# Tai-Wang/Depth-from-Motion

Hardware: AMD Instinct MI355X
Metric: cost-volumes/sec (higher is better)
Workload: dtype bf16; 1 GPU; nstar: plane-sweep cost-volume build B=8/GPU x (2C=512, D=112, 94x311), feats 256x94x311 bf16, fsf=4 csf=1; global_batch=8, parallelism=dp1, kernel=sweep_tile_kernel<LDS>, launch=lanes256_ppl8_planes2_chunk1_pipelined_cut64, autotuned=True, volume_layout=(B,2C,D,H,W) contiguous (the reference layout)

## Files before the change

### depth-from-motion_amd/_capi.py

```python
import ctypes
import os

_HERE = os.path.dirname(os.path.abspath(__file__))
LIB_PATH = os.environ.get('DFM_HIP_LIB', os.path.join(_HERE, 'lib', 'libdfm_hip.so'))

DFM_F32, DFM_BF16 = 0, 1


class SweepDesc(ctypes.Structure):
    _fields_ = [
        ('batch', ctypes.c_int32),
        ('channels', ctypes.c_int32),
        ('h_in', ctypes.c_int32),
        ('w_in', ctypes.c_int32),
        ('num_depths', ctypes.c_int32),
        ('h_out', ctypes.c_int32),
        ('w_out', ctypes.c_int32),
        ('feat_sample_factor', ctypes.c_float),
        ('cost_sample_factor', ctypes.c_float),
        ('img_scale_factor', ctypes.c_float),
        ('crop_x', ctypes.c_float),
        ('crop_y', ctypes.c_float),
        ('org_w', ctypes.c_float),
        ('flip', ctypes.c_int32),
        ('dtype', ctypes.c_int32),
    ]


class SweepOpts(ctypes.Structure):
    _fields_ = [(n, ctypes.c_int32) for n in (
        'kernel', 'lanes_per_workgroup', 'lds_kib', 'blocks_per_group', 'planes_per_workgroup',
        'bands_per_chunk', 'points_per_lane', 'pipeline', 'store_align_points', 'pair_stores',
        'unpack')] + [('reserved', ctypes.c_int32 * 1)]

    def as_dict(self):
        return {n: getattr(self, n) for n, _ in self._fields_ if n != 'reserved'}


class MvDesc(ctypes.Structure):
    _fields_ = [
        ('num_views', ctypes.c_int32),
        ('num_frames', ctypes.c_int32),
        ('channels', ctypes.c_int32),
        ('feat_h', ctypes.c_int32),
        ('feat_w', ctypes.c_int32),
        ('nx', ctypes.c_int32),
        ('ny', ctypes.c_int32),
        ('nz', ctypes.c_int32),
        ('num_points', ctypes.c_int64),
        ('scale_x', ctypes.c_float),
        ('scale_y', ctypes.c_float),
        ('crop_x', ctypes.c_float),
        ('crop_y', ctypes.c_float),
        ('flip', ctypes.c_int32),
        ('pad_h', ctypes.c_float),
        ('pad_w', ctypes.c_float),
        ('mode', ctypes.c_int32),
        ('aggregate', ctypes.c_int32),
        ('valid_sample', ctypes.c_int32),
        ('dtype', ctypes.c_int32),
        ('out_channels_last', ctypes.c_int32),
        ('feats_channels_last', ctypes.c_int32),
    ]


class F2vDesc(ctypes.Structure):
    _fields_ = [(n, ctypes.c_int32) for n in (
        'batch', 'channels', 'd', 'h', 'w', 'ds', 'hs', 'ws', 'sem_channels', 'hsem', 'wsem', 'nz',
        'ny', 'nx')] + [(n, ctypes.c_float) for n in ('pad_h', 'pad_w', 'depth_min', 'depth_span')
# ... 208 lines not shown
    ci, i32, i64, sz, f32, f64 = (ctypes.c_int, ctypes.c_int32, ctypes.c_int64, ctypes.c_size_t, ctypes.c_float,
                                  ctypes.c_double)
    dp, op, mp, f2p, spp, pp = P(SweepDesc), P(SweepOpts), P(MvDesc), P(F2vDesc), P(SppDesc), P(vp)
    vsp, vmp, cp, wp, lp = P(VsDesc), P(VsMvDesc), P(Conv3dDesc), P(Conv3dWgradDesc), P(DepthLossDesc)
    ip, atp, ahp, adp, ddp = P(ImitationDesc), P(AnchorTargetDesc), P(AnchorHeadDesc), P(AtssTargetDesc), P(DeformDesc)
    vdp, sdp, plp, i32p, i64p = P(VoxelDesc), P(SparseConvDesc), P(SparseConvPlan), P(i32), P(i64)
    dtp, alp, slp = P(DepthTargetsDesc), P(AnchorLossDesc), P(AtssLossDesc)
    return {
        'dfm_hip.h': _table(
            ('dfm_version', ci, []),
            ('dfm_last_error', ctypes.c_char_p, []),
            ('dfm_profile_begin', ci, [ci]),
            ('dfm_profile_end', ci, [P(f64), P(ci)]),
            ('dfm_camera_prepare', ci, [fp, i32, i32, i32, fp, fp, vp]),
            ('dfm_plane_sweep_workspace_bytes', sz, [dp]),
            ('dfm_plane_sweep_fwd', ci, [dp, vp, vp, fp, fp, fp, fp, vp, vp, sz, vp]),
            ('dfm_plane_sweep_cl_workspace_bytes', sz, [dp]),
            ('dfm_plane_sweep_fwd_channels_last', ci, [dp, vp, vp, fp, fp, fp, fp, vp, vp, sz, vp]),
            ('dfm_plane_sweep_fwd_nhwc', ci, [dp, vp, vp, fp, fp, fp, fp, vp, vp, sz, vp]),
            ('dfm_plane_sweep_fwd_from_nhwc', ci, [dp, vp, vp, fp, fp, fp, fp, vp, vp, sz, vp]),
            ('dfm_plane_sweep_bwd', ci, [dp, vp, fp, fp, fp, fp, fp, fp, vp]),
            ('dfm_plane_sweep_grid', ci, [dp, i32, fp, fp, fp, fp, fp, fp, vp]),
            ('dfm_plane_sweep_last_kernel', ci, []),
            ('dfm_plane_sweep_bwd_last_kernel', ci, []),
            ('dfm_plane_sweep_fwd_opts', ci, [dp, vp, vp, fp, fp, fp, fp, vp, vp, sz, vp, op]),
            ('dfm_plane_sweep_bwd_opts', ci, [dp, vp, fp, fp, fp, fp, fp, fp, vp, op]),
            ('dfm_plane_sweep_bwd_channels_last', ci, [dp, vp, fp, fp, fp, fp, fp, fp, vp, sz, vp]),
            ('dfm_plane_sweep_bwd_cur_nhwc', ci, [dp, vp, fp, fp, fp, fp, fp, vp]),
            ('dfm_plane_sweep_bwd_prev_gather_workspace_bytes', sz, [dp]),
            ('dfm_plane_sweep_bwd_prev_gather', ci, [dp, vp, fp, fp, fp, fp, fp, vp, sz, vp]),
            ('dfm_plane_sweep_bwd_gather', ci, [dp, i32, vp, i32, fp, fp, fp, fp, fp, i32, vp, sz, vp]),
            ('dfm_plane_sweep_autotune', ci, [dp, vp, vp, fp, fp, fp, fp, vp, vp, sz, vp, op]),
            ('dfm_plane_sweep_tuning', ci, [dp, op]),
            ('dfm_plane_sweep_reset_tuning', None, []),
            ('dfm_store_probe', ci, [vp, i32, i32, i64, i32, i32, vp]),
            ('dfm_clock_probe', ci, [vp, i32, vp]),
            ('dfm_point_sample_mv_workspace_bytes', sz, [mp]),
            ('dfm_point_sample_mv_fwd', ci, [mp, vp, fp, fp, fp, vp, vp, vp, sz, vp]),
            ('dfm_frustum_to_voxel_workspace_bytes', sz, [f2p]),
            ('dfm_frustum_to_voxel_fwd', ci, [f2p, vp, vp, vp, fp, fp, vp, vp, sz, vp]),
            ('dfm_depth_head_fwd', ci, [i32, i32, i32, i32, i32, i32, vp, fp, vp, vp, vp, vp]),
            ('dfm_depth_head_stats_fwd', ci, [i32, i32, i32, i32, i32, i32, vp, fp, fp, fp, vp, vp]),
            ('dfm_frustum_to_voxel_fused_fwd', ci, [f2p, vp, vp, fp, fp, i32, vp, fp, fp, vp, vp, sz, vp]),
            ('dfm_frustum_to_voxel_bwd_workspace_bytes', sz, [f2p]),
            ('dfm_frustum_to_voxel_bwd', ci, [f2p, vp, vp, fp, fp, fp, fp, vp, sz, vp]),
            ('dfm_frustum_to_voxel_fused_bwd', ci, [f2p, vp, vp, fp, fp, i32, fp, fp, fp, fp, vp, sz, vp]),
            ('dfm_frustum_to_voxel_bwd_gather_workspace_bytes', sz, [f2p]),
            ('dfm_frustum_to_voxel_bwd_gather', ci, [f2p, vp, vp, vp, fp, fp, i32, fp, P(f32), fp, fp, fp, vp, sz,
                                                     vp]),
            ('dfm_frustum_to_voxel_bwd_gather_cl', ci, [f2p, vp, vp, vp, fp, fp, i32, fp, P(f32), fp, vp, fp, vp, sz,
                                                        vp]),
            ('dfm_point_sample_mv_fwd_batched', ci, [vp, i32, vp, fp, i32, fp, fp, vp, vp, vp]),
            ('dfm_point_sample_mv_bwd_workspace_bytes', sz, [mp]),
            ('dfm_point_sample_mv_bwd', ci, [mp, vp, fp, fp, fp, fp, vp, sz, vp]),
            ('dfm_depth_head_bwd', ci, [i32, i32, i32, i32, i32, i32, vp, fp, vp, vp, vp, fp, vp]),
            ('dfm_sweep_conv_weight_bytes', sz, []),
            ('dfm_sweep_conv_pack_weights', ci, [vp, vp, i32, vp, vp]),
            ('dfm_sweep_conv_stats_splits', ci, [dp, i32]),
            ('dfm_sweep_conv_fwd', ci, [dp, vp, vp, fp, fp, fp, fp, vp, vp, vp, fp, fp, i32, vp]),
            ('dfm_cost_gate_weight_bytes', sz, [i32]),
            ('dfm_cost_gate_pack_weights', ci, [vp, i32, i32, vp, vp]),
            ('dfm_cost_gate_fwd', ci, [i32, i32, i64, i32, vp, vp, vp, vp, vp]),
            ('dfm_conv3d_k3_c32_weight_bytes', sz, []),
            ('dfm_conv3d_k3_c32_pack_weights', ci, [vp, i32, i32, i32, i32, vp, vp]),
            ('dfm_conv3d_k3_c32_stats_splits', ci, [i32, i32, i32, i32, i32]),
            ('dfm_conv3d_k3_c32_fwd', ci, [i32, i32, i32, i32, vp, vp, fp, vp, i32, i32, i32, fp, vp]),
# ... 179 lines not shown
```

### depth-from-motion_amd/csrc/plane_sweep.hip

```cpp
#include "plane_sweep_common.h"

#include <stdlib.h>
#include <string.h>

#include <algorithm>
#include <map>
#include <mutex>
#include <vector>

using namespace dfm;

namespace {

thread_local int g_last_kernel = 0;
#ifdef DFM_DEBUG_HOOKS
unsigned long long *g_trace = nullptr;
#endif

struct Launch {
    int kernel;
    int lanes;
    int lds_kib;
    int bpg;
    int planes;
    int band_chunk;
    int ppl;
    int align;
    int pair;
    int unpack;
    int pipe;
};

struct TuneKey {
    int v[9];
    bool operator<(const TuneKey &o) const { return memcmp(v, o.v, sizeof(v)) < 0; }
};
std::mutex g_tune_mu;
std::map<TuneKey, dfm_sweep_opts> g_tuned;

constexpr int PACK_PPL = 1;
__global__ void sweep_reset_kernel(int *flags, int n_flags, int *b, int *c)
{
    for (int i = threadIdx.x; i < n_flags; i += blockDim.x) flags[i] = 0;
    if (threadIdx.x == 0) { *b = 0; *c = 0; }
}

template <typename T>
__global__ __launch_bounds__(256) void pack_blocked_kernel(const T *__restrict__ src0,
                                                           const T *__restrict__ src1,
                                                           uint4 *__restrict__ dst0,
                                                           uint4 *__restrict__ dst1, int batch,
                                                           int C, int HW, int nblk, int *__restrict__ flags,
                                                           int W)
{
    constexpr int CB = elem<T>::CB;
    const int pix0 = blockIdx.x * (256 * PACK_PPL) + threadIdx.x;
    const int blk = blockIdx.y;
    const bool second = (int)blockIdx.z >= batch;
// ... 171 lines not shown
        dc += HW;
        dp += HW;
    }
}

typedef uint32_t u32x4_t __attribute__((ext_vector_type(4)));

__device__ __forceinline__ void vol_store16(const u32x4_t &v, void *p)
{
    __builtin_nontemporal_store(v, (u32x4_t *)p);
}

__device__ __forceinline__ constexpr int waitcnt_vm(int n)
{
    return (n & 15) | (7 << 4) | (15 << 8) | ((n >> 4) << 14);
}

__device__ __forceinline__ int swz(int q) { return q ^ ((q >> 4) & 7); }

__device__ __forceinline__ uint32_t footprint(float x, float y, int H, int W, int &rN, int &rS,
                                              int &ix, float &fw, float &fn)
{
    const Tap t = make_tap(x, y, H, W);
    ix = (t.ok & 5u) ? t.ix : t.ix - ((t.ok & 10u) ? 1 : 0);
    rN = t.iy;
    rS = t.iy + t.dy;
    const bool fin = (fabsf(x) <= 3.0e38f) && (fabsf(y) <= 3.0e38f);
    fw = fin ? x - floorf(x) : 0.0f;
    fn = fin ? y - floorf(y) : 0.0f;
    return t.ok;
}

struct TileGrid {
    int batch;
    int bands;
    int band_pts;
    int planes;
    int dgroups;
    int blocks_per_group;
    int band_chunk;
    const int *flags;
    int mfma_unpack;
    int pair_stores;
    int align;
    unsigned long long *trace;
    int ablate;
};

constexpr int PIPE_BUF_SLOTS = 2504;
constexpr int PIPE_LDS_BYTES = (8 + 2 * PIPE_BUF_SLOTS) * 16;
template <int N> struct IntC { static constexpr int value = N; };

template <typename T, int NT, bool LDS, int V, bool PIPE = false, bool MXK = false>
__device__ __forceinline__ int tile_body(
    const int bid, const SweepGeom &g, const SweepFast &fast, const TileGrid &tg, int lds_slots,
    const uint4 *__restrict__ cur_blk, const uint4 *__restrict__ prev_blk,
    const float *__restrict__ depths, const float *__restrict__ P,
    const float *__restrict__ Pinv, const float *__restrict__ Tm, T *__restrict__ out,
    int *__restrict__ spill_list, int blk_lo_ovr = -1, int blk_hi_ovr = -1, bool retry_inline = false)
{
    constexpr int CB = elem<T>::CB;
    static_assert(V == 4 || V == 8, "points per lane");
    static_assert(V * sizeof(T) == 16 || V * sizeof(T) == 8, "8- or 16-byte stores");
    static_assert(LDS || !PIPE, "the pipelined body is an LDS-staged body");
    static_assert(!MXK || (LDS && sizeof(T) == 2 && V == 8), "matrix-core unpack: bf16, LDS taps, 8 points per lane");
    constexpr int VW = V * (int)sizeof(T) / 4;
    constexpr int PAD = 8;
    constexpr int SLAB = 8;
    extern __shared__ __attribute__((aligned(16))) uint4 lds[];
    int *bb = (int *)lds;

    const int tid = threadIdx.x;
    const int batch = tg.batch;
    const int b = bid % batch;
    int th = bid / batch;
    const int band_in = th % tg.band_chunk;
    th /= tg.band_chunk;
    const int dgroup = th % tg.dgroups;
    th /= tg.dgroups;
    const int half = th & 1;
    th >>= 1;
    const int nchunks = (tg.bands + tg.band_chunk - 1) / tg.band_chunk;
    const int band = (th % nchunks) * tg.band_chunk + band_in;
    const int group = th / nchunks;
    if (band >= tg.bands) return 0;
    const int blk_lo = blk_lo_ovr >= 0 ? blk_lo_ovr : group * tg.blocks_per_group;
    const int blk_hi = blk_lo_ovr >= 0 ? min(blk_hi_ovr, g.nblk) : min(blk_lo + tg.blocks_per_group, g.nblk);
    const int lanes_per_plane = NT / tg.planes;
    const int d_tile = dgroup * tg.planes + tid / lanes_per_plane;
    const int tid_p = tid % lanes_per_plane;
    const long long hw_ll = (long long)g.h_out * g.w_out;
    const long long a0 = (d_tile * hw_ll) & ~7ll;
    const long long a1 = d_tile >= g.D - 1 ? g.N : (((d_tile + 1) * hw_ll) & ~7ll);
    const long long base = a0 & ~(long long)(tg.align - 1);
    const long long t_end = d_tile < g.D ? min(base + (long long)(band + 1) * tg.band_pts, a1) : 0;
    const long long n0 = base + (long long)band * tg.band_pts + (long long)tid_p * V;
    const bool active = n0 >= a0 && n0 < t_end;
    const int W = g.w_in, H = g.h_in;
    const int HW = H * W;

    if (LDS) {
        if (tid == 0) {
            bb[0] = 0x7fffffff;
            bb[1] = -1;
            lds[SLAB] = make_uint4(0u, 0u, 0u, 0u);
            if constexpr (PIPE) lds[SLAB + PIPE_BUF_SLOTS] = make_uint4(0u, 0u, 0u, 0u);
        }
        __syncthreads();
    }

    int qN[V], qS[V];
    float fw[V], fn[V];
    uint32_t okbits = 0;
    int ymin = 0x7fffffff, ymax = -1;
    if (active) {
        const int hw = g.h_out * g.w_out;
        int d = (int)(n0 / hw);
        int rem = (int)(n0 - (long long)d * hw);
// ... 603 lines not shown
{
    return (((size_t)2 * d->batch * d->h_in * 4) + 255) & ~(size_t)255;
}

size_t flag_bytes(const dfm_sweep_desc *d)
{
    const int V = d->dtype == DFM_BF16 ? 8 : 4;
    const long long hw = (long long)d->h_out * d->w_out;
    const long long bands = (hw + 7 + 63 + 64ll * V - 1) / (64ll * V);
    const long long nblk = (d->channels + V - 1) / V;
    return ((size_t)(1 + bands * d->num_depths * 2 * d->batch * nblk) * 4 + 255) & ~(size_t)255;
}

SweepFast make_fast(const dfm_sweep_desc *d)
{
    SweepFast fast;
    fast.scale_is_one = d->img_scale_factor == 1.0f;
    int e = 0;
    const float m = frexpf(d->feat_sample_factor, &e);
    fast.fsf_pow2 = (m == 0.5f) && e > -60 && e < 60;
    fast.inv_fsf = 1.0f / d->feat_sample_factor;
    return fast;
}

int resolve(const dfm_sweep_desc *d, const dfm_sweep_opts *o, Launch &L)
{
    const int CB = d->dtype == DFM_BF16 ? 8 : 4;
    L.kernel = o ? o->kernel : 0;
    L.lanes = o && o->lanes_per_workgroup ? o->lanes_per_workgroup : 256;
    L.lds_kib = o && o->lds_kib ? o->lds_kib : 0;
    L.bpg = o && o->blocks_per_group ? o->blocks_per_group : (1 << 20);
    L.planes = o && o->planes_per_workgroup ? o->planes_per_workgroup : 2;
    L.band_chunk = o && o->bands_per_chunk ? o->bands_per_chunk : 1;
    L.ppl = o && o->points_per_lane ? o->points_per_lane : CB;
    L.align = o && o->store_align_points ? o->store_align_points : 64;
    if (L.align != 8 && L.align != 16 && L.align != 32 && L.align != 64)
        return set_error(DFM_ERR_INVALID_ARG, "opts: store_align_points in {8,16,32,64}");
    L.pair = o && o->pair_stores ? (o->pair_stores == 1) : 1;
    if (o && (o->unpack < 0 || o->unpack > 2)) return set_error(DFM_ERR_INVALID_ARG, "opts: unpack must be 0, 1 or 2");
    L.unpack = o && o->unpack ? (o->unpack == 1) : 1;
    L.pipe = o && o->pipeline ? o->pipeline : 2;
    if (L.pipe != 1 && L.pipe != 2) return set_error(DFM_ERR_INVALID_ARG, "opts: pipeline must be 0, 1 or 2");
    if (!L.lds_kib) L.lds_kib = L.pipe >= 2 ? 80 : 52;
    if (L.kernel < 0 || L.kernel > 5) return set_error(DFM_ERR_INVALID_ARG, "opts: kernel must be 0..5");
    if (L.lanes != 128 && L.lanes != 256 && L.lanes != 512 && L.lanes != 1024)
        return set_error(DFM_ERR_INVALID_ARG, "opts: lanes_per_workgroup in {128,256,512,1024}");
    if (L.lds_kib < 4 || L.lds_kib > 160 || L.bpg < 1 || L.planes < 1 || L.band_chunk < 1)
        return set_error(DFM_ERR_INVALID_ARG, "opts: 4 <= lds_kib <= 160, blocks_per_group / planes / bands_per_chunk >= 1");
    if (L.ppl != CB && !(L.ppl == 4 && CB == 8 && L.lanes >= 256))
        return set_error(DFM_ERR_INVALID_ARG, "opts: points_per_lane is 16/sizeof(T), or 4 for bf16 with >= 256 lanes");
    if (L.lanes == 1024 && L.ppl != 4)
        return set_error(DFM_ERR_INVALID_ARG, "opts: 1024 lanes need points_per_lane = 4");
    return DFM_OK;
}

template <typename T, int NT, int V>
int launch_tiles(int which, const dfm_sweep_desc *d, const SweepGeom &g, const Launch &L,
                 const uint4 *cur_blk, const uint4 *prev_blk, const float *depths, const float *P,
                 const float *Pinv, const float *Tm, T *out, int *spill_list, hipStream_t st)
{
    const int lds_bytes = L.lds_kib * 1024;
    const int bpg = which == 2 ? std::min(L.bpg, g.nblk) : g.nblk;
    const int groups = (g.nblk + bpg - 1) / bpg;
    const long long hw = (long long)g.h_out * g.w_out;
    TileGrid tg;
    tg.batch = d->batch;
    tg.planes = std::max(1, std::min(L.planes, NT / 64));
    while ((NT / 64) % tg.planes) --tg.planes;
    tg.dgroups = (g.D + tg.planes - 1) / tg.planes;
    const long long per_plane = (long long)(NT / tg.planes) * V;
    tg.align = (int)std::min<long long>(L.align, per_plane & -per_plane);
    const long long am = tg.align - 1;
    tg.bands = (int)((hw + 7 + am + per_plane - 1) / per_plane);
    tg.band_pts = (int)((((hw + 7 + am + tg.bands - 1) / tg.bands) + am) & ~am);
    tg.blocks_per_group = bpg;
    tg.band_chunk = std::max(1, std::min(L.band_chunk, tg.bands));
    tg.trace = nullptr;
    tg.ablate = 0;
    tg.pair_stores = L.pair;
    tg.mfma_unpack = L.unpack;
    tg.flags = (const int *)((const char *)spill_list + 2 * flag_bytes(d));
#ifdef DFM_DEBUG_HOOKS
    tg.trace = g_trace;
    {
        const char *ab = getenv("DFM_ABLATE");
        tg.ablate = ab ? atoi(ab) : 0;
    }
#endif
    const long long nchunks = (tg.bands + tg.band_chunk - 1) / tg.band_chunk;
    const long long nb = nchunks * tg.band_chunk * tg.dgroups * 2 * d->batch * groups;
    if (nb > 2147483647ll) return set_error(DFM_ERR_UNSUPPORTED, "too many lattice points");
    if ((size_t)(nb + 1) * 4 > flag_bytes(d)) return set_error(DFM_ERR_WORKSPACE, "spill list too small");
    int rc = DFM_OK;
    const SweepFast fast = make_fast(d);
    if (which == 2) {
        int *spill2 = (int *)((char *)spill_list + flag_bytes(d));
        constexpr bool CAN_MX = sizeof(T) == 2 && V == 8;
        if (L.pipe >= 2 && CAN_MX && L.unpack) {
            if constexpr (CAN_MX) {
                const void *kern = (const void *)sweep_tile_kernel<T, NT, true, V, true, true>;
                rc = ensure_dynamic_lds(kern, PIPE_LDS_BYTES);
                if (rc != DFM_OK) return rc;
                hipLaunchKernelGGL((sweep_tile_kernel<T, NT, true, V, true, true>), dim3((unsigned)nb), dim3(NT),
                                   PIPE_LDS_BYTES, st, g, fast, tg, std::min(lds_bytes, PIPE_LDS_BYTES) / 16,
                                   cur_blk, prev_blk, depths, P, Pinv, Tm, out, spill_list);
            }
        } else if (L.pipe >= 2) {
            const void *kern = (const void *)sweep_tile_kernel<T, NT, true, V, true>;
            rc = ensure_dynamic_lds(kern, PIPE_LDS_BYTES);
            if (rc != DFM_OK) return rc;
            hipLaunchKernelGGL((sweep_tile_kernel<T, NT, true, V, true>), dim3((unsigned)nb), dim3(NT),
                               PIPE_LDS_BYTES, st, g, fast, tg, std::min(lds_bytes, PIPE_LDS_BYTES) / 16,
                               cur_blk, prev_blk, depths, P, Pinv, Tm, out, spill_list);
        } else {
            const void *kern = (const void *)sweep_tile_kernel<T, NT, true, V>;
            rc = ensure_dynamic_lds(kern, lds_bytes);
            if (rc != DFM_OK) return rc;
            hipLaunchKernelGGL((sweep_tile_kernel<T, NT, true, V>), dim3((unsigned)nb), dim3(NT),
                               lds_bytes, st, g, fast, tg, lds_bytes / 16, cur_blk, prev_blk, depths, P,
                               Pinv, Tm, out, spill_list);
        }
        const bool queues = !(L.pipe >= 2 && V * sizeof(T) == 16);
        if (queues) {
// ... 97 lines not shown

int check_fwd_args(const dfm_sweep_desc *desc, const void *cur, const void *prev,
                   const float *depths, const float *cam2img, const float *cam2img_inv,
                   const float *cur2prev, void *out, void *workspace, size_t workspace_bytes)
{
    int rc = check_desc(desc);
    if (rc != DFM_OK) return rc;
    if (!cur || !prev || !depths || !cam2img || !cam2img_inv || !cur2prev || !out)
        return set_error(DFM_ERR_INVALID_ARG, "NULL device pointer");
    if (!workspace || workspace_bytes < fwd_workspace_bytes(desc))
        return set_error(DFM_ERR_WORKSPACE, "workspace smaller than dfm_plane_sweep_workspace_bytes");
    if (((uintptr_t)workspace & 15) || ((uintptr_t)out & 1))
        return set_error(DFM_ERR_INVALID_ARG, "workspace must be 16-byte aligned");
    return DFM_OK;
}

int tune_key(const dfm_sweep_desc *d, TuneKey &k)
{
    int dev = 0;
    HIP_TRY(hipGetDevice(&dev));
    const int v[9] = {dev, d->batch, d->channels, d->h_in, d->w_in, d->num_depths, d->h_out,
                      d->w_out, d->dtype};
    memcpy(k.v, v, sizeof(v));
    return DFM_OK;
}

bool takes_lds_tiles(const dfm_sweep_desc *d, const void *out)
{
    const int CB = d->dtype == DFM_BF16 ? 8 : 4;
    const long long N = (long long)d->num_depths * d->h_out * d->w_out;
    return N % CB == 0 && ((uintptr_t)out & 15) == 0 && d->cost_sample_factor < 1.5f;
}

}

int dfm::sweep_check_desc(const dfm_sweep_desc *d) { return check_desc(d); }
dfm::SweepGeom dfm::sweep_make_geom(const dfm_sweep_desc *d) { return make_geom(d); }
dfm::SweepFast dfm::sweep_make_fast(const dfm_sweep_desc *d) { return make_fast(d); }
void dfm::sweep_set_last_kernel(int which) { g_last_kernel = which; }
int dfm::sweep_bwd_scatter_launch(const dfm_sweep_desc *desc, const void *grad_out, const float *depths,
                                  const float *cam2img, const float *cam2img_inv, const float *cur2prev,
                                  float *grad_cur, float *grad_prev, void *stream)
{
    const SweepGeom g = make_geom(desc);
    hipStream_t st = (hipStream_t)stream;
    const long long nb = (g.N + 255) / 256;
    if (nb > 2147483647ll) return set_error(DFM_ERR_UNSUPPORTED, "too many lattice points");
    dim3 grid((unsigned)nb, desc->batch);
    by_dtype(desc->dtype, [&](auto t) {
        using T = decltype(t);
        hipLaunchKernelGGL(sweep_bwd_kernel<T>, grid, dim3(256), 0, st, g, (const T *)grad_out, depths, cam2img,
                           cam2img_inv, cur2prev, grad_cur, grad_prev);
    });
    return DFM_OK;
}

extern "C" {

DFM_API int dfm_plane_sweep_last_kernel(void) { return g_last_kernel; }
#ifdef DFM_DEBUG_HOOKS
DFM_API void dfm_debug_set_trace(void *buf) { g_trace = (unsigned long long *)buf; }
#endif

DFM_API int dfm_camera_prepare(const float *cam2img, int32_t rows, int32_t cols, int32_t batch,
                               float *cam2img_4x4, float *cam2img_inv, void *stream)
{
// ... 56 lines not shown

DFM_API int dfm_plane_sweep_fwd(const dfm_sweep_desc *desc, const void *cur, const void *prev,
                                const float *depths, const float *cam2img,
                                const float *cam2img_inv, const float *cur2prev, void *out,
                                void *workspace, size_t workspace_bytes, void *stream)
{
    return dfm_plane_sweep_fwd_opts(desc, cur, prev, depths, cam2img, cam2img_inv, cur2prev, out,
                                    workspace, workspace_bytes, stream, nullptr);
}

DFM_API int dfm_plane_sweep_autotune(const dfm_sweep_desc *desc, const void *cur, const void *prev,
                                     const float *depths, const float *cam2img,
                                     const float *cam2img_inv, const float *cur2prev, void *out,
                                     void *workspace, size_t workspace_bytes, void *stream,
                                     dfm_sweep_opts *chosen)
{
    int rc = check_fwd_args(desc, cur, prev, depths, cam2img, cam2img_inv, cur2prev, out, workspace,
                            workspace_bytes);
    if (rc != DFM_OK) return rc;
    TuneKey key;
    rc = tune_key(desc, key);
    if (rc != DFM_OK) return rc;
    std::vector<dfm_sweep_opts> cand;
    {
        dfm_sweep_opts o;
        memset(&o, 0, sizeof(o));
        o.bands_per_chunk = 1;
        cand.push_back(o);
        if (desc->dtype == DFM_BF16) {
            o.lanes_per_workgroup = 512;
            o.points_per_lane = 4;
            cand.push_back(o);
        }
    }
    hipStream_t st = (hipStream_t)stream;
    dfm_sweep_opts best = cand[0];
    if (takes_lds_tiles(desc, out)) {
        constexpr int ROUNDS = 4, PER = 2;
        hipEvent_t e0, e1;
        HIP_TRY(hipEventCreate(&e0));
        HIP_TRY(hipEventCreate(&e1));
        std::vector<Launch> Ls(cand.size());
        for (size_t i = 0; i < cand.size() && rc == DFM_OK; ++i) rc = resolve(desc, &cand[i], Ls[i]);
        for (size_t i = 0; i < cand.size() && rc == DFM_OK; ++i)
            rc = run_fwd(desc, Ls[i], cur, prev, depths, cam2img, cam2img_inv, cur2prev, out, workspace, st);
        for (int w = 0; w < 2 && rc == DFM_OK; ++w)
            rc = run_fwd(desc, Ls[0], cur, prev, depths, cam2img, cam2img_inv, cur2prev, out, workspace, st);
        std::vector<float> tmin(cand.size(), 3.0e38f);
        std::vector<std::vector<float>> rounds(cand.size());
        for (int r = 0; r < ROUNDS && rc == DFM_OK; ++r)
            for (size_t i = 0; i < cand.size() && rc == DFM_OK; ++i) {
                (void)hipEventRecord(e0, st);
                for (int k = 0; k < PER && rc == DFM_OK; ++k)
                    rc = run_fwd(desc, Ls[i], cur, prev, depths, cam2img, cam2img_inv, cur2prev, out,
                                 workspace, st);
                (void)hipEventRecord(e1, st);
                if (rc == DFM_OK && hipEventSynchronize(e1) != hipSuccess)
                    rc = set_error(DFM_ERR_HIP, "autotune: event sync failed");
                float ms = 0.0f;
                if (rc == DFM_OK) (void)hipEventElapsedTime(&ms, e0, e1);
                if (rc == DFM_OK) rounds[i].push_back(ms);
            }
        for (size_t i = 0; i < cand.size() && rc == DFM_OK; ++i) {
            std::sort(rounds[i].begin(), rounds[i].end());
            tmin[i] = rounds[i][rounds[i].size() / 2];
        }
        (void)hipEventDestroy(e0);
        (void)hipEventDestroy(e1);
        if (rc != DFM_OK) return rc;
        size_t bi = 0;
        for (size_t i = 1; i < cand.size(); ++i) {
            const float margin = cand[i].bands_per_chunk > 1 && cand[bi].bands_per_chunk <= 1 ? 0.985f : 1.0f;
            if (tmin[i] < tmin[bi] * margin) bi = i;
        }
        best = cand[bi];
    } else {
        Launch L;
        rc = resolve(desc, nullptr, L);
        if (rc == DFM_OK)
            rc = run_fwd(desc, L, cur, prev, depths, cam2img, cam2img_inv, cur2prev, out, workspace, st);
        if (rc != DFM_OK) return rc;
    }
    {
        std::lock_guard<std::mutex> lk(g_tune_mu);
        g_tuned[key] = best;
    }
    if (chosen) *chosen = best;
    return DFM_OK;
}

DFM_API int dfm_plane_sweep_tuning(const dfm_sweep_desc *desc, dfm_sweep_opts *opts)
{
    int rc = check_desc(desc);
    if (rc != DFM_OK) return rc;
    if (!opts) return set_error(DFM_ERR_INVALID_ARG, "NULL output");
    TuneKey k;
    rc = tune_key(desc, k);
    if (rc != DFM_OK) return rc;
    memset(opts, 0, sizeof(*opts));
    std::lock_guard<std::mutex> lk(g_tune_mu);
    auto it = g_tuned.find(k);
    if (it == g_tuned.end()) return 0;
    *opts = it->second;
    return 1;
}

DFM_API void dfm_plane_sweep_reset_tuning(void)
{
    std::lock_guard<std::mutex> lk(g_tune_mu);
    g_tuned.clear();
}

DFM_API int dfm_plane_sweep_grid(const dfm_sweep_desc *desc, int32_t b, const float *depths,
                                 const float *cam2img, const float *cam2img_inv,
                                 const float *cur2prev, float *cur_grid, float *prev_grid,
                                 void *stream)
{
    int rc = check_desc(desc);
    if (rc != DFM_OK) return rc;
    if (b < 0 || b >= desc->batch) return set_error(DFM_ERR_INVALID_ARG, "sample index out of range");
    if (!depths || !cam2img || !cam2img_inv || !cur2prev || !cur_grid || !prev_grid)
        return set_error(DFM_ERR_INVALID_ARG, "NULL device pointer");
    const SweepGeom g = make_geom(desc);
    const long long nb = (g.N + 255) / 256;
    if (nb > 2147483647ll) return set_error(DFM_ERR_UNSUPPORTED, "too many lattice points");
    hipLaunchKernelGGL(sweep_grid_kernel, dim3((unsigned)nb), dim3(256), 0, (hipStream_t)stream, g,
                       b, depths, cam2img, cam2img_inv, cur2prev, cur_grid, prev_grid);
    HIP_TRY(hipGetLastError());
    return DFM_OK;
}

}
```

### depth-from-motion_amd/csrc/plane_sweep_common.h

```cpp
#pragma once
#include "dfm_common.h"

namespace dfm {

struct SweepGeom;
struct SweepFast;
int sweep_check_desc(const dfm_sweep_desc *d);
SweepGeom sweep_make_geom(const dfm_sweep_desc *d);
void sweep_set_last_kernel(int which);
SweepFast sweep_make_fast(const dfm_sweep_desc *d);
int sweep_bwd_scatter_launch(const dfm_sweep_desc *desc, const void *grad_out, const float *depths,
                             const float *cam2img, const float *cam2img_inv, const float *cur2prev,
                             float *grad_cur, float *grad_prev, void *stream);
void sweep_set_last_bwd_kernel(int which);
bool sweep_clt_supported(const dfm_sweep_desc *d, const void *out);
size_t sweep_clt_workspace_bytes(const dfm_sweep_desc *d);
int sweep_clt_launch(const dfm_sweep_desc *d, const void *cur, const void *prev, const float *depths,
                     const float *cam2img, const float *cam2img_inv, const float *cur2prev, void *out,
                     void *workspace, void *stream, bool nhwc = false, bool walk = true);
bool sweep_cltw_supported(const dfm_sweep_desc *d, const void *out);
bool sweep_bwd_mfma_supported(const dfm_sweep_desc *d, const void *grad_out);
int sweep_bwd_mfma_launch(const dfm_sweep_desc *d, int half, const void *grad_out, const float *depths,
                          const float *P, const float *Pinv, const float *Tm, float *grad_cur, float *grad_prev,
                          void *stream);
constexpr float SWEEP_BWD_ZOOM_ONE = 1.4f, SWEEP_BWD_ZOOM_TWO = 2.75f, SWEEP_BWD_ZOOM_FOUR = 3.9f;

struct SweepGeom {
    int32_t C, h_in, w_in, D, h_out, w_out;
    int32_t nblk;
    int32_t flip;
    float fsf, csf, scale, crop_x, crop_y, org_w;
    long long N;
};

// ... 179 lines not shown
```

### depth-from-motion_amd/plane_sweep.py

```python
import contextlib
import os
import ctypes
import threading

import numpy as np
import torch

from . import _capi
from ._launch import DTYPES, STREAM, WS, launch, require_gpu, try_launch, upload


def _pad4x4_batch(m, batch_size):
    m = m[:batch_size]
    rows = 3 if m.shape[-2] == 4 else m.shape[-2]
    out = torch.eye(4, dtype=torch.float32, device=m.device).repeat(batch_size, 1, 1)
    out[:, :rows, :m.shape[-1]] = m[:, :rows]
    return out


def camera_matrices(cam2imgs, cur2prevs, batch_size, device, cam2img_inv=None):
    def as_f32(x):
        if isinstance(x, (list, tuple)):
            if len(x) and torch.is_tensor(x[0]):
                x = torch.stack(list(x))
# ... 18 lines not shown
        Pinv = torch.stack([torch.inverse(P[i]) for i in range(batch_size)])
    if cur2prevs.device.type == 'cuda':
        pack = upload(torch.stack([P, Pinv]).reshape(2, batch_size, 16), device)
        return pack[0], pack[1], cur2prevs[:batch_size].to(device).reshape(batch_size, 16).contiguous()
    T = cur2prevs[:batch_size]
    pack = upload(torch.stack([P, Pinv, T]).reshape(3, batch_size, 16), device)
    return pack[0], pack[1], pack[2]


def _make_desc(cur_feats, num_depths, feat_sample_factor, cost_sample_factor, img_shape, flip,
               img_crop_offset, img_scale_factor):
    batch_size, channels, h_in, w_in = cur_feats.shape
    desc = _capi.SweepDesc()
    desc.batch, desc.channels, desc.h_in, desc.w_in = batch_size, channels, h_in, w_in
    desc.num_depths = num_depths
    desc.h_out = round(h_in / cost_sample_factor)
    desc.w_out = round(w_in / cost_sample_factor)
    desc.feat_sample_factor = float(feat_sample_factor)
    desc.cost_sample_factor = float(cost_sample_factor)
    desc.img_scale_factor = float(img_scale_factor)
    desc.crop_x = float(img_crop_offset[0])
    desc.crop_y = float(img_crop_offset[1])
    desc.org_w = float(img_shape[1])
    desc.flip = 1 if flip else 0
    desc.dtype = DTYPES[cur_feats.dtype]
    return desc


_tls = threading.local()
_OPT_FIELDS = {'kernel': 'kernel', 'lanes': 'lanes_per_workgroup', 'lds_kib': 'lds_kib',
               'blocks_per_group': 'blocks_per_group', 'planes': 'planes_per_workgroup',
               'bands_per_chunk': 'bands_per_chunk', 'points_per_lane': 'points_per_lane',
               'pipeline': 'pipeline', 'store_align': 'store_align_points',
               'pair_stores': 'pair_stores', 'unpack': 'unpack'}


def make_opts(**kw):
    o = _capi.SweepOpts()
    for k, v in kw.items():
        setattr(o, _OPT_FIELDS[k], int(v or 0))
    return o


@contextlib.contextmanager
def launch_options(**kw):
    prev = getattr(_tls, 'opts', None)
    _tls.opts = make_opts(**kw) if kw else None
    try:
        yield _tls.opts
    finally:
        _tls.opts = prev


_PREV_GATHER = {'on': os.environ.get('DFM_NO_PREV_GATHER') != '1'}


@contextlib.contextmanager
def prev_gather(on):
    prev, _PREV_GATHER['on'] = _PREV_GATHER['on'], bool(on)
    try:
        yield
    finally:
        _PREV_GATHER['on'] = prev


_bwd_kernel = None
_bwd_kernel_lock = threading.RLock()
# ... 48 lines not shown
                      STREAM, ws_bytes=256 + 4 * desc.channels):
            return out
    cur_feats, prev_feats = cur_feats.contiguous(), prev_feats.contiguous()
    if channels_last:
        if out is None:
            out = torch.empty((desc.batch, desc.num_depths, desc.h_out, desc.w_out, 2 * desc.channels),
                              dtype=cur_feats.dtype, device=device).permute(0, 4, 1, 2, 3)
        assert out.is_contiguous(memory_format=torch.channels_last_3d)
        launch('dfm_plane_sweep_fwd_channels_last', desc, cur_feats, prev_feats, depths, P, Pinv, T, out, WS,
               STREAM, ws_bytes=lib.dfm_plane_sweep_cl_workspace_bytes(ctypes.byref(desc)))
        return out
    if out is None:
        out = torch.empty((desc.batch, 2 * desc.channels, desc.num_depths, desc.h_out, desc.w_out),
                          dtype=cur_feats.dtype, device=device)
    launch('dfm_plane_sweep_fwd_opts', desc, cur_feats, prev_feats, depths, P, Pinv, T, out, WS, STREAM,
           _current_opts(schedule), ws_bytes=lib.dfm_plane_sweep_workspace_bytes(ctypes.byref(desc)))
    return out


def plane_sweep_autotune(desc, cur_feats, prev_feats, depths, P, Pinv, T, out):
    chosen = _capi.SweepOpts()
    launch('dfm_plane_sweep_autotune', desc, cur_feats, prev_feats, depths, P, Pinv, T, out, WS, STREAM, chosen,
           ws_bytes=_capi.lib().dfm_plane_sweep_workspace_bytes(ctypes.byref(desc)))
    return chosen.as_dict()


def plane_sweep_tuning(desc):
    lib = _capi.lib()
    o = _capi.SweepOpts()
    rc = lib.dfm_plane_sweep_tuning(ctypes.byref(desc), ctypes.byref(o))
    if rc < 0:
        _capi.check(rc)
    return o.as_dict() if rc == 1 else None


class _PlaneSweepFn(torch.autograd.Function):

    @staticmethod
    def forward(ctx, cur_feats, prev_feats, depths, P, Pinv, T, desc, channels_last=False):
        ctx.desc = desc
        ctx.save_for_backward(depths, P, Pinv, T)
        ctx.in_dtype = cur_feats.dtype
        return plane_sweep_forward(desc, cur_feats, prev_feats, depths, P, Pinv, T,
                                   channels_last=channels_last)

    @staticmethod
    def backward(ctx, grad_out):
        depths, P, Pinv, T = ctx.saved_tensors
        g_cur, g_prev = plane_sweep_backward(ctx.desc, grad_out, depths, P, Pinv, T)
        return g_cur.to(ctx.in_dtype), g_prev.to(ctx.in_dtype), None, None, None, None, None, None


def plane_sweep_backward(desc, grad_out, depths, P, Pinv, T):
    lib = _capi.lib()
    device = grad_out.device
    require_gpu(grad_out, 'grad_out')
    shape = (desc.batch, desc.channels, desc.h_in, desc.w_in)
    opts = _current_opts()
    if _bwd_kernel is not None:
        opts = make_opts(kernel=_bwd_kernel)
    if (opts is None and not grad_out.is_contiguous() and grad_out.dim() == 5 and
            grad_out.is_contiguous(memory_format=torch.channels_last_3d)):
        if (_PREV_GATHER['on'] and desc.cost_sample_factor >= 1.5 and desc.channels % 32 == 0 and
                DTYPES.get(grad_out.dtype) == desc.dtype):
            nb = lib.dfm_plane_sweep_bwd_prev_gather_workspace_bytes(ctypes.byref(desc))
            maps = [torch.empty((desc.batch, desc.h_in, desc.w_in, desc.channels), dtype=torch.float32,
# ... 79 lines not shown
```

### include/dfm_hip.h

```cpp
#ifndef DFM_HIP_H
#define DFM_HIP_H

#include <stddef.h>
#include <stdint.h>

#ifdef __cplusplus
extern "C" {
#endif

#define DFM_API __attribute__((visibility("default")))

typedef enum dfm_status {
    DFM_OK = 0,
    DFM_ERR_INVALID_ARG = -1,
    DFM_ERR_UNSUPPORTED = -2,
    DFM_ERR_WORKSPACE = -3,
    DFM_ERR_HIP = -4
} dfm_status;

typedef enum dfm_dtype { DFM_F32 = 0, DFM_BF16 = 1 } dfm_dtype;

DFM_API int dfm_version(void);
DFM_API const char *dfm_last_error(void);

// ... 74 lines not shown
                                     const float *depths, const float *cam2img,
                                     const float *cam2img_inv, const float *cur2prev, void *out,
                                     void *workspace, size_t workspace_bytes, void *stream,
                                     const dfm_sweep_opts *opts);
DFM_API int dfm_plane_sweep_bwd_opts(const dfm_sweep_desc *desc, const void *grad_out,
                                     const float *depths, const float *cam2img,
                                     const float *cam2img_inv, const float *cur2prev,
                                     float *grad_cur, float *grad_prev, void *stream,
                                     const dfm_sweep_opts *opts);
DFM_API int dfm_plane_sweep_bwd_channels_last(const dfm_sweep_desc *desc, const void *grad_out,
                                              const float *depths, const float *cam2img,
                                              const float *cam2img_inv, const float *cur2prev,
                                              float *grad_cur, float *grad_prev, void *workspace,
                                              size_t workspace_bytes, void *stream);
DFM_API int dfm_plane_sweep_bwd_cur_nhwc(const dfm_sweep_desc *desc, const void *grad_out, const float *depths,
                                         const float *cam2img, const float *cam2img_inv,
                                         const float *cur2prev, float *grad_cur, void *stream);
DFM_API size_t dfm_plane_sweep_bwd_prev_gather_workspace_bytes(const dfm_sweep_desc *desc);
DFM_API int dfm_plane_sweep_bwd_gather(const dfm_sweep_desc *desc, int32_t half, const void *grad_out,
                                       int32_t grad_channels_last, const float *depths, const float *cam2img,
                                       const float *cam2img_inv, const float *cur2prev, float *grad_map,
                                       int32_t map_pixel_major, void *workspace, size_t workspace_bytes,
                                       void *stream);
DFM_API int dfm_plane_sweep_bwd_prev_gather(const dfm_sweep_desc *desc, const void *grad_out, const float *depths,
                                            const float *cam2img, const float *cam2img_inv,
                                            const float *cur2prev, float *grad_prev, void *workspace,
                                            size_t workspace_bytes, void *stream);
DFM_API int dfm_plane_sweep_autotune(const dfm_sweep_desc *desc, const void *cur, const void *prev,
                                     const float *depths, const float *cam2img,
                                     const float *cam2img_inv, const float *cur2prev, void *out,
                                     void *workspace, size_t workspace_bytes, void *stream,
                                     dfm_sweep_opts *chosen);
DFM_API int dfm_plane_sweep_tuning(const dfm_sweep_desc *desc, dfm_sweep_opts *opts);
DFM_API int dfm_store_probe(void *out, int32_t batch, int32_t planes, int64_t plane_bytes, int32_t run_bytes,
                            int32_t planes_per_workgroup, void *stream);

DFM_API int dfm_clock_probe(void *out3, int32_t iterations, void *stream);
DFM_API void dfm_plane_sweep_reset_tuning(void);


typedef struct dfm_mv_desc {
    int32_t num_views;
    int32_t num_frames;
    int32_t channels;
    int32_t feat_h, feat_w;
    int32_t nx, ny, nz;
    int64_t num_points;
    float scale_x, scale_y;
    float crop_x, crop_y;
    int32_t flip;
    float pad_h, pad_w;
    int32_t mode;
    int32_t aggregate;
    int32_t valid_sample;
    int32_t dtype;
    int32_t out_channels_last;
    int32_t feats_channels_last;
} dfm_mv_desc;

DFM_API size_t dfm_point_sample_mv_workspace_bytes(const dfm_mv_desc *desc);

DFM_API int dfm_point_sample_mv_fwd(const dfm_mv_desc *desc, const void *feats,
                                    const float *points, const float *proj, const float *ori_w,
                                    void *out, unsigned char *valid, void *workspace,
                                    size_t workspace_bytes, void *stream);
DFM_API int dfm_point_sample_mv_fwd_batched(const dfm_mv_desc *descs, int32_t batch, const void *feats,
// ... 442 lines not shown
```

Before: 1613 cost-volumes/s.

## Add selectable tile-order schedule for plane-sweep workgroup decomposition

Moves the decoding of workgroup id into (batch, half, depth-group, band, group) into a shared schedule header with three selectable orders for where the cur/prev half index sits. Order 0 matches the old decomposition, so the default path is unchanged. The autotuner now filters candidates with an admission rule on live working-set size and drops the margin that favoured multi-band chunks. It also exposes a query API for the resulting plan. Other orders are meant to improve L2 reuse of the source feature blocks across concurrently running workgroups, but no new order candidates are added to the tuner here.

```diff
diff --git a/depth-from-motion_amd/_capi.py b/depth-from-motion_amd/_capi.py
--- a/depth-from-motion_amd/_capi.py
+++ b/depth-from-motion_amd/_capi.py
@@ -33,8 +33,10 @@
         'bands_per_chunk', 'points_per_lane', 'pipeline', 'store_align_points', 'pair_stores',
         'unpack')] + [('reserved', ctypes.c_int32 * 1)]
 
+    order = property(lambda self: self.reserved[0], lambda self, v: self.reserved.__setitem__(0, v))
+
     def as_dict(self):
-        return {n: getattr(self, n) for n, _ in self._fields_ if n != 'reserved'}
+        return dict({n: getattr(self, n) for n, _ in self._fields_ if n != 'reserved'}, order=self.order)
 
 
 class MvDesc(ctypes.Structure):
@@ -309,6 +311,7 @@
             ('dfm_plane_sweep_bwd_gather', ci, [dp, i32, vp, i32, fp, fp, fp, fp, fp, i32, vp, sz, vp]),
             ('dfm_plane_sweep_autotune', ci, [dp, vp, vp, fp, fp, fp, fp, vp, vp, sz, vp, op]),
             ('dfm_plane_sweep_tuning', ci, [dp, op]),
+            ('dfm_plane_sweep_schedule', ci, [dp, op, i64p]),
             ('dfm_plane_sweep_reset_tuning', None, []),
             ('dfm_store_probe', ci, [vp, i32, i32, i64, i32, i32, vp]),
             ('dfm_clock_probe', ci, [vp, i32, vp]),
diff --git a/depth-from-motion_amd/csrc/plane_sweep.hip b/depth-from-motion_amd/csrc/plane_sweep.hip
--- a/depth-from-motion_amd/csrc/plane_sweep.hip
+++ b/depth-from-motion_amd/csrc/plane_sweep.hip
@@ -24,6 +24,7 @@
     int bpg;
     int planes;
     int band_chunk;
+    int order;
     int ppl;
     int align;
     int pair;
@@ -261,13 +262,10 @@
 }
 
 struct TileGrid {
-    int batch;
-    int bands;
+    SweepSchedule sched;
     int band_pts;
     int planes;
-    int dgroups;
     int blocks_per_group;
-    int band_chunk;
     const int *flags;
     int mfma_unpack;
     int pair_stores;
@@ -300,19 +298,10 @@
     int *bb = (int *)lds;
 
     const int tid = threadIdx.x;
-    const int batch = tg.batch;
-    const int b = bid % batch;
-    int th = bid / batch;
-    const int band_in = th % tg.band_chunk;
-    th /= tg.band_chunk;
-    const int dgroup = th % tg.dgroups;
-    th /= tg.dgroups;
-    const int half = th & 1;
-    th >>= 1;
-    const int nchunks = (tg.bands + tg.band_chunk - 1) / tg.band_chunk;
-    const int band = (th % nchunks) * tg.band_chunk + band_in;
-    const int group = th / nchunks;
-    if (band >= tg.bands) return 0;
+    const SweepTileId tile = sweep_schedule_tile(tg.sched, bid);
+    const int batch = tg.sched.batch;
+    const int b = tile.b, half = tile.half, dgroup = tile.dgroup, band = tile.band, group = tile.group;
+    if (band >= tg.sched.bands) return 0;
     const int blk_lo = blk_lo_ovr >= 0 ? blk_lo_ovr : group * tg.blocks_per_group;
     const int blk_hi = blk_lo_ovr >= 0 ? min(blk_hi_ovr, g.nblk) : min(blk_lo + tg.blocks_per_group, g.nblk);
     const int lanes_per_plane = NT / tg.planes;
@@ -982,6 +971,8 @@
     L.bpg = o && o->blocks_per_group ? o->blocks_per_group : (1 << 20);
     L.planes = o && o->planes_per_workgroup ? o->planes_per_workgroup : 2;
     L.band_chunk = o && o->bands_per_chunk ? o->bands_per_chunk : 1;
+    L.order = o ? o->reserved[0] : 0;
+    if (L.order < 0 || L.order >= SWEEP_ORDERS) return set_error(DFM_ERR_INVALID_ARG, "opts: order must be 0, 1 or 2");
     L.ppl = o && o->points_per_lane ? o->points_per_lane : CB;
     L.align = o && o->store_align_points ? o->store_align_points : 64;
     if (L.align != 8 && L.align != 16 && L.align != 32 && L.align != 64)
@@ -1004,31 +995,40 @@
     return DFM_OK;
 }
 
+TileGrid make_tile_grid(int which, const dfm_sweep_desc *d, const SweepGeom &g, const Launch &L, int NT, int V)
+{
+    const int bpg = which == 2 ? std::min(L.bpg, g.nblk) : g.nblk;
+    const long long hw = (long long)g.h_out * g.w_out;
+    TileGrid tg;
+    tg.sched.batch = d->batch;
+    tg.planes = std::max(1, std::min(L.planes, NT / 64));
+    while ((NT / 64) % tg.planes) --tg.planes;
+    tg.sched.dgroups = (g.D + tg.planes - 1) / tg.planes;
+    const long long per_plane = (long long)(NT / tg.planes) * V;
+    tg.align = (int)std::min<long long>(L.align, per_plane & -per_plane);
+    const long long am = tg.align - 1;
+    tg.sched.bands = (int)((hw + 7 + am + per_plane - 1) / per_plane);
+    tg.band_pts = (int)((((hw + 7 + am + tg.sched.bands - 1) / tg.sched.bands) + am) & ~am);
+    tg.blocks_per_group = bpg;
+    tg.sched.groups = (g.nblk + bpg - 1) / bpg;
+    tg.sched.band_chunk = std::max(1, std::min(L.band_chunk, tg.sched.bands));
+    tg.sched.order = L.order;
+    tg.trace = nullptr;
+    tg.ablate = 0;
+    tg.pair_stores = L.pair;
+    tg.mfma_unpack = L.unpack;
+    tg.flags = nullptr;
+    return tg;
+}
+
 template <typename T, int NT, int V>
 int launch_tiles(int which, const dfm_sweep_desc *d, const SweepGeom &g, const Launch &L,
                  const uint4 *cur_blk, const uint4 *prev_blk, const float *depths, const float *P,
                  const float *Pinv, const float *Tm, T *out, int *spill_list, hipStream_t st)
 {
     const int lds_bytes = L.lds_kib * 1024;
-    const int bpg = which == 2 ? std::min(L.bpg, g.nblk) : g.nblk;
-    const int groups = (g.nblk + bpg - 1) / bpg;
     const long long hw = (long long)g.h_out * g.w_out;
-    TileGrid tg;
-    tg.batch = d->batch;
-    tg.planes = std::max(1, std::min(L.planes, NT / 64));
-    while ((NT / 64) % tg.planes) --tg.planes;
-    tg.dgroups = (g.D + tg.planes - 1) / tg.planes;
-    const long long per_plane = (long long)(NT / tg.planes) * V;
-    tg.align = (int)std::min<long long>(L.align, per_plane & -per_plane);
-    const long long am = tg.align - 1;
-    tg.bands = (int)((hw + 7 + am + per_plane - 1) / per_plane);
-    tg.band_pts = (int)((((hw + 7 + am + tg.bands - 1) / tg.bands) + am) & ~am);
-    tg.blocks_per_group = bpg;
-    tg.band_chunk = std::max(1, std::min(L.band_chunk, tg.bands));
-    tg.trace = nullptr;
-    tg.ablate = 0;
-    tg.pair_stores = L.pair;
-    tg.mfma_unpack = L.unpack;
+    TileGrid tg = make_tile_grid(which, d, g, L, NT, V);
     tg.flags = (const int *)((const char *)spill_list + 2 * flag_bytes(d));
 #ifdef DFM_DEBUG_HOOKS
     tg.trace = g_trace;
@@ -1037,8 +1037,7 @@
         tg.ablate = ab ? atoi(ab) : 0;
     }
 #endif
-    const long long nchunks = (tg.bands + tg.band_chunk - 1) / tg.band_chunk;
-    const long long nb = nchunks * tg.band_chunk * tg.dgroups * 2 * d->batch * groups;
+    const long long nb = sweep_schedule_blocks(tg.sched);
     if (nb > 2147483647ll) return set_error(DFM_ERR_UNSUPPORTED, "too many lattice points");
     if ((size_t)(nb + 1) * 4 > flag_bytes(d)) return set_error(DFM_ERR_WORKSPACE, "spill list too small");
     int rc = DFM_OK;
@@ -1202,6 +1201,14 @@
     return N % CB == 0 && ((uintptr_t)out & 15) == 0 && d->cost_sample_factor < 1.5f;
 }
 
+bool candidate_admitted(const dfm_sweep_desc *d, const dfm_sweep_opts *o)
+{
+    const int CB = d->dtype == DFM_BF16 ? 8 : 4;
+    const int nblk = (d->channels + CB - 1) / CB;
+    return sweep_schedule_admitted(nblk, o->blocks_per_group ? o->blocks_per_group : nblk,
+                                   o->bands_per_chunk ? o->bands_per_chunk : 1, o->reserved[0]);
+}
+
 }
 
 int dfm::sweep_check_desc(const dfm_sweep_desc *d) { return check_desc(d); }
@@ -1324,6 +1331,9 @@
             o.points_per_lane = 4;
             cand.push_back(o);
         }
+        cand.erase(std::remove_if(cand.begin() + 1, cand.end(),
+                                  [&](const dfm_sweep_opts &c) { return !candidate_admitted(desc, &c); }),
+                   cand.end());
     }
     hipStream_t st = (hipStream_t)stream;
     dfm_sweep_opts best = cand[0];
@@ -1361,10 +1371,8 @@
         (void)hipEventDestroy(e1);
         if (rc != DFM_OK) return rc;
         size_t bi = 0;
-        for (size_t i = 1; i < cand.size(); ++i) {
-            const float margin = cand[i].bands_per_chunk > 1 && cand[bi].bands_per_chunk <= 1 ? 0.985f : 1.0f;
-            if (tmin[i] < tmin[bi] * margin) bi = i;
-        }
+        for (size_t i = 1; i < cand.size(); ++i)
+            if (tmin[i] < tmin[bi]) bi = i;
         best = cand[bi];
     } else {
         Launch L;
@@ -1403,6 +1411,25 @@
     g_tuned.clear();
 }
 
+DFM_API int dfm_plane_sweep_schedule(const dfm_sweep_desc *desc, const dfm_sweep_opts *opts, int64_t *plan8)
+{
+    int rc = check_desc(desc);
+    if (rc != DFM_OK) return rc;
+    if (!plan8) return set_error(DFM_ERR_INVALID_ARG, "NULL output");
+    Launch L;
+    rc = resolve(desc, opts, L);
+    if (rc != DFM_OK) return rc;
+    const SweepGeom g = make_geom(desc);
+    const TileGrid tg = make_tile_grid(2, desc, g, L, L.lanes, L.ppl);
+    dfm_sweep_opts zero;
+    memset(&zero, 0, sizeof(zero));
+    const int64_t v[8] = {sweep_schedule_blocks(tg.sched), tg.sched.batch, tg.sched.bands, tg.sched.band_chunk,
+                          tg.sched.dgroups, tg.sched.groups, tg.sched.order,
+                          candidate_admitted(desc, opts ? opts : &zero) ? 1 : 0};
+    memcpy(plan8, v, sizeof(v));
+    return DFM_OK;
+}
+
 DFM_API int dfm_plane_sweep_grid(const dfm_sweep_desc *desc, int32_t b, const float *depths,
                                  const float *cam2img, const float *cam2img_inv,
                                  const float *cur2prev, float *cur_grid, float *prev_grid,
diff --git a/depth-from-motion_amd/csrc/plane_sweep_common.h b/depth-from-motion_amd/csrc/plane_sweep_common.h
--- a/depth-from-motion_amd/csrc/plane_sweep_common.h
+++ b/depth-from-motion_amd/csrc/plane_sweep_common.h
@@ -1,5 +1,6 @@
 #pragma once
 #include "dfm_common.h"
+#include "plane_sweep_schedule.h"
 
 namespace dfm {
 
diff --git a/depth-from-motion_amd/csrc/plane_sweep_schedule.h b/depth-from-motion_amd/csrc/plane_sweep_schedule.h
--- /dev/null
+++ b/depth-from-motion_amd/csrc/plane_sweep_schedule.h
@@ -0,0 +1,70 @@
+#pragma once
+
+#if defined(__HIPCC__)
+#define DFM_SCHED_FN __host__ __device__ inline
+#else
+#define DFM_SCHED_FN inline
+#endif
+
+namespace dfm {
+
+struct SweepSchedule {
+    int batch;
+    int bands;
+    int band_chunk;
+    int dgroups;
+    int groups;
+    int order;
+};
+
+struct SweepTileId {
+    int b, half, dgroup, band, group;
+};
+
+constexpr int SWEEP_ORDERS = 3;
+
+DFM_SCHED_FN int sweep_schedule_chunks(const SweepSchedule &s) { return (s.bands + s.band_chunk - 1) / s.band_chunk; }
+
+DFM_SCHED_FN long long sweep_schedule_blocks(const SweepSchedule &s)
+{
+    return (long long)sweep_schedule_chunks(s) * s.band_chunk * s.dgroups * 2 * s.batch * s.groups;
+}
+
+DFM_SCHED_FN SweepTileId sweep_schedule_tile(const SweepSchedule &s, int bid)
+{
+    SweepTileId t;
+    const int nchunks = sweep_schedule_chunks(s);
+    int th = bid;
+    t.b = th % s.batch;
+    th /= s.batch;
+    if (s.order == 2) {
+        t.half = th & 1;
+        th >>= 1;
+    }
+    const int band_in = th % s.band_chunk;
+    th /= s.band_chunk;
+    t.dgroup = th % s.dgroups;
+    th /= s.dgroups;
+    if (s.order == 0) {
+        t.half = th & 1;
+        th >>= 1;
+    }
+    t.band = (th % nchunks) * s.band_chunk + band_in;
+    th /= nchunks;
+    if (s.order == 1) {
+        t.half = th & 1;
+        th >>= 1;
+    }
+    t.group = th;
+    return t;
+}
+
+DFM_SCHED_FN bool sweep_schedule_admitted(int nblk, int blocks_per_group, int bands_per_chunk, int order)
+{
+    if (nblk < 1 || blocks_per_group < 1 || bands_per_chunk < 1 || order < 0 || order >= SWEEP_ORDERS) return false;
+    const long long bpg = blocks_per_group < nblk ? blocks_per_group : nblk;
+    const long long live = (long long)bands_per_chunk * bpg * (order == 1 ? 1 : 2);
+    return live <= 2ll * (2ll * nblk);
+}
+
+}
diff --git a/depth-from-motion_amd/plane_sweep.py b/depth-from-motion_amd/plane_sweep.py
--- a/depth-from-motion_amd/plane_sweep.py
+++ b/depth-from-motion_amd/plane_sweep.py
@@ -74,7 +74,7 @@
                'blocks_per_group': 'blocks_per_group', 'planes': 'planes_per_workgroup',
                'bands_per_chunk': 'bands_per_chunk', 'points_per_lane': 'points_per_lane',
                'pipeline': 'pipeline', 'store_align': 'store_align_points',
-               'pair_stores': 'pair_stores', 'unpack': 'unpack'}
+               'pair_stores': 'pair_stores', 'unpack': 'unpack', 'order': 'order'}
 
 
 def make_opts(**kw):
@@ -189,6 +189,13 @@
     if rc < 0:
         _capi.check(rc)
     return o.as_dict() if rc == 1 else None
+
+
+def plane_sweep_schedule(desc, **kw):
+    plan = (ctypes.c_int64 * 8)()
+    _capi.check(_capi.lib().dfm_plane_sweep_schedule(ctypes.byref(desc), ctypes.byref(make_opts(**kw)), plan))
+    names = ('workgroups', 'batch', 'bands', 'band_chunk', 'dgroups', 'groups', 'order')
+    return dict(zip(names, plan[:7]), admitted=bool(plan[7]))
 
 
 class _PlaneSweepFn(torch.autograd.Function):
diff --git a/include/dfm_hip.h b/include/dfm_hip.h
--- a/include/dfm_hip.h
+++ b/include/dfm_hip.h
@@ -130,6 +130,7 @@
                                      void *workspace, size_t workspace_bytes, void *stream,
                                      dfm_sweep_opts *chosen);
 DFM_API int dfm_plane_sweep_tuning(const dfm_sweep_desc *desc, dfm_sweep_opts *opts);
+DFM_API int dfm_plane_sweep_schedule(const dfm_sweep_desc *desc, const dfm_sweep_opts *opts, int64_t *plan8);
 DFM_API int dfm_store_probe(void *out, int32_t batch, int32_t planes, int64_t plane_bytes, int32_t run_bytes,
                             int32_t planes_per_workgroup, void *stream);
 
```

New measurement: 1608 cost-volumes/s, median of 2. Within noise of the previous version (-0.3%).
